# sean-lo/OptimalMatrixCompletion.jl

Hardware: AMD Instinct MI355X
Metric: B&B node-relaxations/sec, 100x100 k=1 (higher is better)
Workload: dtype f64

## Files before the change

### optimalmatrixcompletion.jl_amd/csrc/omc_device.h

```cpp
#ifndef OMC_DEVICE_H
#define OMC_DEVICE_H
#include <hip/hip_runtime.h>
#include <stdint.h>

#define ROW_TRACE 0
#define ROW_BOX 1
#define ROW_BOUND 2
#define ROW_CUT 3

#define CONE_CLIP01 0
#define CONE_EVALS 2
#define CONE_SEP 3
#define CONE_TOPK 4
#define CONE_BIG 5
#define SMALL_PROJ 0
#define SMALL_RECOVER 1

#define OMC_ST_OPTIMAL 0
#define OMC_ST_SLOW 1
#define OMC_ST_TIME 2
#define OMC_ST_INFEASIBLE 3

#include "omc_layout.h"

struct OmcWS {
  int nB;
  int B, Btot, n, m, k, nnz, Rmax, Lmax, breakpoints, rmax, stall_checks, np16, max_sweeps, max_iters;
  int *node_of, *init, *fin;
  const int* slot_list;
  int check_every, early_stop_after; double early_stop_factor;
  double *gap_prev, *gap_rate; int* slow_votes;
  const double* rho_node;
  double *oY, *oU, *oalphaX, *obx, *oobj, *olb, *olmin, *orho; int *ostatus, *oiters;
  double gamma, rho, rho_f_ratio, relax, eps_gap, eps_feas, sumA2;
  double* rho_b;
  double* bfac;
  int *nbump, *lastbump;
  int bump_max, bump_after, bump_gap; double bump_ratio, bump_factor;
  const int* col_ptr;
  const int* col_idx;
  const double* col_val;
  const double* Ncnt;
  const int* row_ptr;
  const int* row_idx;
  double* lamD;
  double* lamDX;
  const double* wY1;
  double *Y, *Yp;
  double* U;
  double *D1, *D3;
  double *W1, *E3;
  int* w1_fac;
  int skip_yp;
  double* Qb;
  int* rr;
  double *Vt, *D3V, *W3V, *Q3V;
  double *D3T, *W3T, *Q3T;
  double* dS;
  double *alpha, *alphaX;
  double* sval;
  double *objcol, *c0col;
  double* Mchk;
  int check_xs;
  double *Mbuf, *Vrow;
  double* fro2;
  int* vvalid;
  double *MbufC, *VrowC, *fro2c; int* vvalidC; int ws_mode;
  int sub_enable, sub_qmax, sub_chunk, sub_debug; double sub_tol, sub_adapt;
  double* sub_zscratch;
  double* Xs;
  double* sub_theta;
  double* trM;
  double* V3; int* v3valid;
  int *sub_wait, *sub_nfail;
  int *sub_on, *cone_done;
  int* ws_first; int ws_phase;
  int* ws_need;
  int sub_guard;
  int* sep_done;
  int cert_enable; double *XsC, *sub_thetaC, *trMc, *lb_est; int *sub_onC, *confirm;
  int shor;
  int shN;
  const double *shP0, *shD0;
  double clip_hi;
  double inv_s2;
  const int *load_from, *save_to;
  double *pY, *pD1, *pD3, *pU, *palpha, *psval, *pXs, *ptheta, *pscal;
  int mw_budget; int* mw_stat; double* ev_out;
  int* pmw_stat;
  int* sub_stat;
  int* R;
  int *rkind, *rcut, *rbi, *rbj;
  double* rcoef;
  double* rrhs;
  double* cutx;
  double* G;
  int setup_gram_inline;
  double* lam;
  double *obj, *objout, *objprev, *lbprev, *lb, *c0, *evsum, *cpen, *cst, *rp, *rd, *lmin;
  double* bx;
  int *done, *status, *iters, *sweeps, *stall;
  int* rowov;
  OmcGeom geo;
  double* cp_scratch;
  int cp_pair; int cp_nsolo; const int* cp_solo;
  int cp_nwide; const int* cp_wide;
  int cp_nrest;
  int cp_nblock, cp_nslab; const int *cp_block, *cp_slab; const unsigned char* cp_isblock; double* cp_bslab; int* cp_nfact;
  double* Yx;
  int cone_512;
  int cp_series;
  int cp_maxpass;
  int cp_xcd;
  double *cone_scratch, *glob_scratch, *small_scratch;
  double* chk_scratch;
  double* stamps;
  int accel, aa_mem, aa_every, aa_start, aa_dim;
  double aa_reg, aa_safeguard;
  double *aa_F, *aa_G, *aa_zin;
  double* aa_fn;
  int *aa_hist, *aa_head, *aa_pending, *aa_valid, *aa_nacc, *aa_nrej;
  int *cert_flag, *cert_have;
  double *cb_rho, *cbLam, *cblam, *cbPsi, *cbBound;
  double *ocLam, *oclam, *ocPsi, *ocBound; int* ocHave;
};
// ... 45 lines not shown
```

### optimalmatrixcompletion.jl_amd/csrc/omc_device.hip

```cpp
#include <hip/hip_runtime.h>
#include <type_traits>
#include <stdint.h>
#include "omc_device.h"
#include "omc.h"

#include "omc_wave.h"


#ifdef OMC_STAMPS
#define STAMP(slot) do { __syncthreads(); if (blockIdx.x == 0 && threadIdx.x == 0) { long long t_ = __builtin_amdgcn_s_memtime(); w.stamps[slot] += (double)(t_ - t_prev_); t_prev_ = t_; } } while (0)
#define STAMP_BEGIN() long long t_prev_ = __builtin_amdgcn_s_memtime()
#define DIAG_T0() long long t_diag0_ = __builtin_amdgcn_s_memtime()
#define DIAG_ADD(cls, b, v) atomicAdd(&w.stamps[32 + (size_t)(cls) * w.B + (b)], (double)(v))
#define DIAG_CYC(cls, b) DIAG_ADD(cls, b, __builtin_amdgcn_s_memtime() - t_diag0_)
#define WSTAMP_BEGIN() long long tw_prev_ = __builtin_amdgcn_s_memtime()
#define WSTAMP_BEGIN2() tw_prev_ = __builtin_amdgcn_s_memtime()
#define WSTAMP(slot) do { if (b == 0 && j == 0 && lane == 0) { long long t_ = __builtin_amdgcn_s_memtime(); w.stamps[slot] += (double)(t_ - tw_prev_); tw_prev_ = t_; } } while (0)
#else
#define WSTAMP_BEGIN() do {} while (0)
#define WSTAMP_BEGIN2() do {} while (0)
#define WSTAMP(slot) do {} while (0)
#define STAMP(slot) do {} while (0)
#define STAMP_BEGIN() do {} while (0)
#define DIAG_T0() do {} while (0)
// ... 1485 lines not shown
    while ((r + 1) * (r + 2) / 2 <= tile) ++r;
    ti[t] = r; tj[t] = tile - r * (r + 1) / 2;
    const int ia = (ti[t] << 4) + li, jb = (tj[t] << 4) + li;
    ma[t] = (ia < n) ? 1.0 : 0.0; mb[t] = (jb < n) ? 1.0 : 0.0;
    La[t] = L + ((ia < n) ? ia : n - 1);
    Lb[t] = L + ((jb < n) ? jb : n - 1);
    acc[t] = double4v{0.0, 0.0, 0.0, 0.0};
  }
  if (m4 >= 16) {
#pragma unroll
    for (int t = 0; t < NT; ++t)
#pragma unroll
      for (int u = 0; u < 4; ++u) { aq[t][u] = La[t][(size_t)(4 * u + lk) * n]; bq[t][u] = Lb[t][(size_t)(4 * u + lk) * n]; }
  }
  int k0 = 0;
  for (; k0 + 16 <= m4; k0 += 16) {
#pragma unroll
    for (int u = 0; u < 4; ++u) {
      int kn = k0 + 16 + 4 * u + lk;
      kn = (kn < m4) ? kn : kn - 16;
#pragma unroll
      for (int t = 0; t < NT; ++t) {
        const double a = aq[t][u] * ma[t], bv = bq[t][u] * mb[t];
        aq[t][u] = La[t][(size_t)kn * n]; bq[t][u] = Lb[t][(size_t)kn * n];
        acc[t] = __builtin_amdgcn_mfma_f64_16x16x4f64(a, bv, acc[t], 0, 0, 0);
      }
    }
  }
  for (; k0 < m; k0 += 4) {
    const int kk = k0 + lk;
#pragma unroll
    for (int t = 0; t < NT; ++t) {
      const double a = (kk < m) ? La[t][(size_t)kk * n] * ma[t] : 0.0, bv = (kk < m) ? Lb[t][(size_t)kk * n] * mb[t] : 0.0;
      acc[t] = __builtin_amdgcn_mfma_f64_16x16x4f64(a, bv, acc[t], 0, 0, 0);
    }
  }
#pragma unroll
  for (int t = 0; t < NT; ++t)
#pragma unroll
    for (int r = 0; r < 4; ++r) {
      const int i = (ti[t] << 4) + lk + 4 * r, j = (tj[t] << 4) + li;
      if (i < n && j < n && i >= j) store(i, j, acc[t][r]);
    }
}
template <int NT, class StoreF>
__device__ __forceinline__ void mfma_LLt(const double* L, int n, int m, StoreF store) {
  const int tid = threadIdx.x, wv = tid >> 6, lane = tid & 63, nw = blockDim.x >> 6, li = lane & 15, lk = lane >> 4;
  const int nt = (n + 15) >> 4, ntile = nt * (nt + 1) / 2;
  int tile = wv;
  for (; tile + (NT - 1) * nw < ntile; tile += NT * nw) mfma_LLt_tiles<NT>(L, n, m, tile, nw, li, lk, store);
  if constexpr (NT > 1) for (; tile < ntile; tile += nw) mfma_LLt_tiles<1>(L, n, m, tile, nw, li, lk, store);
}

template <bool USE_LDS>
__global__ void __launch_bounds__(256) k_small(OmcWS w, int mode) {
  extern __shared__ double smem[];
  __shared__ double red[32];
  __shared__ int s_cnt, s_nsel;
  __shared__ double s_base;
  const int b = slot_of(w, blockIdx.x), tid = threadIdx.x, T = blockDim.x;
  if (w.done[b] && mode == SMALL_PROJ) return;
  if (mode == SMALL_RECOVER && !w.fin[b]) return;
  const int nb = w.node_of[b];
  const int n = w.n, k = w.k, rm = w.rmax;
  const int r = w.rr[nb];
  const int N3 = (mode == SMALL_PROJ) ? r + k : r;
  const int Np = (N3 + 1) & ~1, ld = Np | 1;
  auto base = [&]() { if constexpr (USE_LDS) return (double*)smem; else return w.small_scratch + (size_t)b * w.geo.small.slab_stride; }();
  const SmallLayout L = small_layout(n, rm, k);
  const int ld3 = L.ld3;
  double* T1 = base;
  double* M3 = base + L.M3;
  double *Gm = base + L.Gm, *ev = base + L.ev, *wgt = base + L.wgt;
  int* sel = (int*)(base + L.sel);
  double* Cc = base + L.Cc;
  double* Qs = base + L.Qs;
  const double* Q = w.Qb + (size_t)nb * n * rm;
  const double* Y = w.Y + (size_t)b * n * n;
  const double* D3 = w.D3 + (size_t)b * n * n;
  const double* Vt = w.Vt + (size_t)b * rm * k;
  STAMP_BEGIN();
  DIAG_T0();
  constexpr int T1_RS = 16;
  if (USE_LDS && r <= T1_RS && n <= T) {
    for (int e = tid; e < n * T1_RS; e += T) { const int j = e / T1_RS, a = e % T1_RS; Qs[e] = (a < r) ? Q[(size_t)a * n + j] : 0.0; }
    __syncthreads();
    {
      const int wv_ = tid >> 6, lane_ = tid & 63, li = lane_ & 15, lk = lane_ >> 4, nt = (n + 15) >> 4, nw_ = T >> 6;
      const bool proj = (mode == SMALL_PROJ);
      for (int ti = wv_; ti < nt; ti += nw_) {
        const int ia = (ti << 4) + li; const bool va = ia < n; const int iac = va ? ia : 0;
        double4v acc = {0.0, 0.0, 0.0, 0.0};
        double ya[4], da[4];
#pragma unroll
        for (int u = 0; u < 4; ++u) { const int kk = 4 * u + lk, kc = (kk < n) ? kk : 0; ya[u] = Y[(size_t)kc * n + iac]; da[u] = proj ? D3[(size_t)kc * n + iac] : 0.0; }
        for (int k0 = 0; k0 < n; k0 += 16) {
#pragma unroll
          for (int u = 0; u < 4; ++u) {
            const int kk = k0 + 4 * u + lk; const bool vk = kk < n;
            const double av = ya[u] - da[u], bv = Qs[(vk ? kk : 0) * T1_RS + li];
            const int kn = kk + 16, knc = (kn < n) ? kn : 0;
            ya[u] = Y[(size_t)knc * n + iac]; da[u] = proj ? D3[(size_t)knc * n + iac] : 0.0;
            acc = __builtin_amdgcn_mfma_f64_16x16x4f64((va && vk) ? av : 0.0, vk ? bv : 0.0, acc, 0, 0, 0);
          }
        }
#pragma unroll
        for (int r4 = 0; r4 < 4; ++r4) {
          const int row = (ti << 4) + lk + 4 * r4;
          if (row < n && li < r) T1[(size_t)li * n + row] = acc[r4];
        }
      }
      __syncthreads();
    }
  } else {
    for (int e = tid; e < n * r; e += T) {
      int i = e % n, a = e / n;
      double acc = 0.0;
      if (mode == SMALL_PROJ) for (int j = 0; j < n; ++j) acc += (Y[(size_t)j * n + i] - D3[(size_t)j * n + i]) * Q[(size_t)a * n + j];
      else for (int j = 0; j < n; ++j) acc += Y[(size_t)j * n + i] * Q[(size_t)a * n + j];
      T1[(size_t)a * n + i] = acc;
    }
    __syncthreads();
  }
  STAMP(16);
  for (int e = tid; e < N3 * N3; e += T) {
    int i = e % N3, j = e / N3;
    double v;
    if (i < r && j < r) { v = 0.0; for (int t = 0; t < n; ++t) v += Q[(size_t)i * n + t] * T1[(size_t)j * n + t]; }
    else if (i < r) v = Vt[(size_t)(j - r) * rm + i] - w.D3V[(size_t)b * rm * k + (size_t)(j - r) * rm + i];
    else if (j < r) v = Vt[(size_t)(i - r) * rm + j] - w.D3V[(size_t)b * rm * k + (size_t)(i - r) * rm + j];
    else v = ((i == j) ? 1.0 : 0.0) - w.D3T[(size_t)b * k * k + (size_t)(j - r) * k + (i - r)];
    M3[(size_t)j * ld3 + i] = v;
  }
  __syncthreads();
  STAMP(17);
  if (N3 == 0) return;
// ... 47 lines not shown
        for (int c2 = 0; c2 < r; ++c2) dot += gt[c2] * Vt[(size_t)j * rm + c2];
        acc += wgt[s] * gt[a] * dot;
      }
      Cc[(size_t)j * rm + a] = acc;
    }
    __syncthreads();
    for (int e = tid; e < n * k; e += T) {
      int i = e % n, j = e / n;
      double acc = 0.0;
      for (int a = 0; a < r; ++a) acc += T1[(size_t)a * n + i] * Cc[(size_t)j * rm + a];
      w.U[(size_t)b * n * k + e] = acc;
    }
    return;
  }
  STAMP(18);
  if (tid == 0) {
    int npos = 0, nneg = 0;
    for (int t = 0; t < N3; ++t) { double lamv = sqrt(ev[t]) - sigma; if (lamv > 0.0) ++npos; else if (lamv < 0.0) ++nneg; }
    const bool use_neg = nneg <= npos;
    int c = 0;
    for (int t = 0; t < N3; ++t) {
      double nu2 = ev[t], lamv = sqrt(nu2) - sigma;
      if (use_neg ? (lamv < 0.0) : (lamv > 0.0)) { sel[c] = t; wgt[c] = fabs(lamv) / nu2; ++c; }
    }
    s_nsel = c; s_base = use_neg ? 1.0 : 0.0;
  }
  __syncthreads();
  const bool acc_is_Q3 = (s_base == 1.0);
  double* dS = w.dS + (size_t)b * rm * rm;
  auto store = [&](int i, int j, double v, double Mv) {
    double accv = v - s_base * Mv;
    double q3 = acc_is_Q3 ? accv : (accv - Mv);
    double p3 = acc_is_Q3 ? (Mv + accv) : accv;
    if (i < r && j < r) { dS[(size_t)j * rm + i] = q3; dS[(size_t)i * rm + j] = q3; }
    else if (i >= r && j < r) {
      w.W3V[(size_t)b * rm * k + (size_t)(i - r) * rm + j] = p3;
      w.Q3V[(size_t)b * rm * k + (size_t)(i - r) * rm + j] = q3;
    } else if (i >= r && j >= r) {
      w.W3T[(size_t)b * k * k + (size_t)(j - r) * k + (i - r)] = p3; w.W3T[(size_t)b * k * k + (size_t)(i - r) * k + (j - r)] = p3;
      w.Q3T[(size_t)b * k * k + (size_t)(j - r) * k + (i - r)] = q3; w.Q3T[(size_t)b * k * k + (size_t)(i - r) * k + (j - r)] = q3;
    }
  };
  spectral_rebuild(Gm, ld, N3, sel, wgt, s_nsel, s_base, entry, store);
  __syncthreads();
  __threadfence_block();
  STAMP(19);
  for (int e = tid; e < n * r; e += T) {
    int i = e % n, a = e / n;
    double acc = 0.0;
    for (int c2 = 0; c2 < r; ++c2) acc += Q[(size_t)c2 * n + i] * dS[(size_t)a * rm + c2];
    T1[(size_t)a * n + i] = acc;
  }
  __syncthreads();
  double* E3 = w.E3 + (size_t)b * n * n;
  if (USE_LDS && r <= 16 && n <= T) {
    const int wv_ = tid >> 6, lane_ = tid & 63, li = lane_ & 15, lk = lane_ >> 4, nt = (n + 15) >> 4, nw_ = T >> 6;
    for (int tile = wv_; tile < nt * nt; tile += nw_) {
      const int ti = tile / nt, tj = tile - ti * nt;
      const int ia = (ti << 4) + li, jb = (tj << 4) + li;
      const bool va = ia < n, vb = jb < n;
      const int iac = va ? ia : 0, jbc = vb ? jb : 0;
      double4v acc = {0.0, 0.0, 0.0, 0.0};
#pragma unroll
      for (int k0 = 0; k0 < 16; k0 += 4) {
        const int a = k0 + lk; const bool vk = a < r;
        const double av = T1[(size_t)(vk ? a : 0) * n + iac], bv = Qs[jbc * 16 + a];
        acc = __builtin_amdgcn_mfma_f64_16x16x4f64((va && vk) ? av : 0.0, vb ? bv : 0.0, acc, 0, 0, 0);
      }
#pragma unroll
      for (int r4 = 0; r4 < 4; ++r4) {
        const int row = (ti << 4) + lk + 4 * r4, col = (tj << 4) + li;
        if (row < n && col < n) E3[(size_t)row * n + col] = acc[r4];
      }
    }
  } else {
    for (int e = tid; e < n * n; e += T) {
      int i = e % n, j = e / n;
      if (i < j) continue;
      double acc = 0.0;
      for (int a = 0; a < r; ++a) acc += T1[(size_t)a * n + i] * Q[(size_t)a * n + j];
      E3[(size_t)j * n + i] = acc; E3[(size_t)i * n + j] = acc;
    }
  }
  STAMP(20);
  if (tid == 0) DIAG_CYC(5, b);
}

__device__ __forceinline__ double w1_entry(const double* Xf, const double* wf, int nf, int n, int i, int j) {
  const int p = (i > j) ? i : j, q = (i > j) ? j : i;
  double acc = 0.0;
  for (int c = 0; c < nf; ++c) { const double* x = Xf + (size_t)c * n; acc += x[p] * (x[q] * wf[c]); }
  return acc;
}

template <bool USE_LDS>
__global__ void __launch_bounds__(512) k_global(OmcWS w) {
  extern __shared__ double smem[];
  __shared__ double red[32];
  __shared__ double s_Gp[NNQP_GP_DOUBLES];
  __shared__ double s_sv[NNQP_PMAX], s_tmp[NNQP_PMAX];
  __shared__ int s_pl[NNQP_PMAX];
  const int b = slot_of(w, blockIdx.x), tid = threadIdx.x, T = blockDim.x;
  if (w.done[b]) return;
  const int nb = w.node_of[b];
  const int n = w.n, k = w.k, m = w.m, rm = w.rmax;
  const GlobLayout L = glob_layout(n, k, rm, w.Rmax);
// ... 1115 lines not shown
```

### optimalmatrixcompletion.jl_amd/csrc/omc_host.h

```cpp
#pragma once
#include <hip/hip_runtime.h>
#include <stdint.h>
#include <atomic>
#include <mutex>
#include <string>
#include <thread>
#include <unordered_map>
#include <vector>

#include "omc.h"
#include "omc_carve.h"
#include "omc_device.h"
#include "omc_shor_relax.h"
#include "omc_shor_index.h"
#include "omc_walks.h"

extern thread_local std::string g_err;
static inline int fail(int code, const std::string& msg) { g_err = msg; return code; }
#define HIPCHK(x)                                                                                         \
  do {                                                                                                    \
    hipError_t e_ = (x);                                                                                  \
    if (e_ != hipSuccess) {                                                                               \
      g_err = std::string(#x) + ": " + hipGetErrorString(e_);                                             \
      return (int)e_ > 0 ? (int)e_ : 999;                                                                 \
// ... 40 lines not shown
  field = (T*)b.p;
  return 0;
}
template <class T> static inline int bind(DevBuf& b, T*& field, size_t count, hipStream_t zero_on) {
  const int rc = bind(b, field, count);
  if (rc) return rc;
  HIPCHK(hipMemsetAsync(b.p, 0, count * sizeof(T), zero_on));
  return 0;
}
#define BIND(...) do { int r_ = bind(__VA_ARGS__); if (r_) return r_; } while (0)

struct PinBuf {
  void* p = nullptr; size_t cap = 0;
  PinBuf() = default;
  PinBuf(const PinBuf&) = delete;
  PinBuf& operator=(const PinBuf&) = delete;
  ~PinBuf() { if (p) (void)hipHostFree(p); }
  int ensure(size_t bytes) {
    if (bytes <= cap) return 0;
    if (p) (void)hipHostFree(p);
    p = nullptr; cap = 0;
    hipError_t e = hipHostMalloc(&p, bytes, hipHostMallocDefault);
    if (e != hipSuccess) { g_err = std::string("hipHostMalloc: ") + hipGetErrorString(e); return (int)e; }
    cap = bytes;
    return 0;
  }
  template <class T> T* as() { return (T*)p; }
};

struct Tuning {
  bool altmin_nolds = false;
  bool colprox_no_xcd = false;
  bool cone_512 = false;
  bool dense_proj = false;
  bool host_phases = false;
  bool global_nolds = false;
  bool no_colprox_pair = false;
  bool no_graph = false;
  bool no_subspace = false;
  bool no_ws_split = false;
  bool segv_trace = false;
  bool setup_gram_inline = false;
  bool shor_explicit = false;
  bool shor_no_subspace = false;
  int check_xs = 16;
  int colprox_block_min = 65;
  int cone_multi_min = 1025;
  int event_merge = 1;
  int graph_max = 16;
  int harvest_async = 1;
  int harvest_async_min_live = 256;
  int plain_multi_min = 1025;
  int shor_index_device_min = 0;
  int shor_select_kb = 1048576;
  int streams = 4;
  int sub_debug = 0;
  int sub_qmax = 24;
  int timing_stride = 1;
  int ws_quiet = 1;
};
struct Knob { const char* name; bool Tuning::*flag; int Tuning::*num; };
inline const Knob OMC_KNOBS[] = {
  {"OMC_ALTMIN_NOLDS", &Tuning::altmin_nolds, nullptr},      {"OMC_COLPROX_NO_XCD", &Tuning::colprox_no_xcd, nullptr},
  {"OMC_CONE_512", &Tuning::cone_512, nullptr},              {"OMC_DENSE_PROJ", &Tuning::dense_proj, nullptr},
  {"OMC_GLOBAL_NOLDS", &Tuning::global_nolds, nullptr},      {"OMC_HOST_PHASES", &Tuning::host_phases, nullptr},
  {"OMC_NO_COLPROX_PAIR", &Tuning::no_colprox_pair, nullptr},
  {"OMC_NO_GRAPH", &Tuning::no_graph, nullptr},              {"OMC_NO_SUBSPACE", &Tuning::no_subspace, nullptr},
  {"OMC_NO_WS_SPLIT", &Tuning::no_ws_split, nullptr},        {"OMC_SEGV_TRACE", &Tuning::segv_trace, nullptr},
  {"OMC_SETUP_GRAM_INLINE", &Tuning::setup_gram_inline, nullptr},
  {"OMC_SHOR_EXPLICIT", &Tuning::shor_explicit, nullptr},    {"OMC_SHOR_NO_SUBSPACE", &Tuning::shor_no_subspace, nullptr},
  {"OMC_COLPROX_BLOCK_MIN", nullptr, &Tuning::colprox_block_min},
  {"OMC_CHECK_XS", nullptr, &Tuning::check_xs},              {"OMC_CONE_MULTI_MIN", nullptr, &Tuning::cone_multi_min},
  {"OMC_EVENT_MERGE", nullptr, &Tuning::event_merge},
  {"OMC_GRAPH_MAX", nullptr, &Tuning::graph_max},            {"OMC_SHOR_SELECT_KB", nullptr, &Tuning::shor_select_kb},
  {"OMC_SHOR_INDEX_DEVICE_MIN", nullptr, &Tuning::shor_index_device_min},
  {"OMC_HARVEST_ASYNC", nullptr, &Tuning::harvest_async},    {"OMC_HARVEST_ASYNC_MIN_LIVE", nullptr, &Tuning::harvest_async_min_live},
  {"OMC_WS_QUIET", nullptr, &Tuning::ws_quiet},
  {"OMC_STREAMS", nullptr, &Tuning::streams},                {"OMC_PLAIN_MULTI_MIN", nullptr, &Tuning::plain_multi_min},
  {"OMC_SUB_DEBUG", nullptr, &Tuning::sub_debug},            {"OMC_SUB_QMAX", nullptr, &Tuning::sub_qmax},
  {"OMC_TIMING_STRIDE", nullptr, &Tuning::timing_stride},
};

struct omc_instance {
  int n = 0, m = 0, k = 0, device = 0, nnz = 0, cmax = 0;
  double gamma = 0, sumA2 = 0;
  std::vector<int> col_ptr, col_idx; std::vector<double> col_val;
  std::vector<double> A; std::vector<uint8_t> mask;
  std::vector<double> Ncnt;
  std::vector<int> row_ptr, row_idx; std::vector<double> row_val;
  DevBuf drow_ptr, drow_idx, drow_val, aR, arkind, arcut, arbi, arbj, arcoef, arrhs, acutx, aU0, aU, aV, aobj, aint, aG, aG2;
  hipStream_t stream = nullptr;
  Tuning tun;
  hipStream_t gs[3] = {};
  hipEvent_t gev[5] = {};
  hipEvent_t gevc[5] = {};
  hipEvent_t ev_main = nullptr;
  PinBuf pin_flags[2], pin_list[2], pin_done, pin_jobs; DevBuf bgramjobs;
  hipEvent_t ev_up[4] = {}; bool ev_up_rec[4] = {}; hipEvent_t ev_gram = nullptr; bool ev_gram_rec = false;
  double host_ms[OMC_HOST_NPHASE] = {0}; int64_t host_cnt[OMC_HOST_NPHASE] = {0};
  DevBuf dA, dmask, dcol_ptr, dcol_idx, dcol_val, dNcnt, dwY, dsolo, dwide;
  int nwide = 0;
  int nsolo = 0;
  DevBuf dblock, dslab, disblock, bcpb, bnfact;
  int nblock = 0, nslab = 0, nrest = 0, cpb_cl = 0, cpb_cs = 0, crest_max = 0;
  bool lists_valid = false; int lists_block_min = 0; bool lists_pair = true;
  DevBuf bYx, bY, bYp, bU, bD1, bD3, bW1, bE3, bQb, brr, bsm, bdS, balpha, balphaX, bsval, bMchk, bsmall, bchk;
  DevBuf bR, brkind, brcut, brbi, brbj, brcoef, brrhs, bcutx, bG, blam;
  DevBuf bobjcol, baaF, baaG, baaZ, baaS, baaI, bMbufC, bVrowC, bchkS, bchkI;
  DevBuf bslotlist, bgap, bvotes, blamDX, bXsC, bsubSC, bsubIC;
  DevBuf bsubz, bscal, bbx, bint, bcp, bcone, bglob, bXout, bThout, bXin, bMbuf, bVrow, bXs, bsubS, bsubI;
  long long sub_tot[8] = {0};
  DevBuf bmwstat, sbigmw, pjM, pjV, pjW, pjS, pjD, pjI;
  long long mw_tot[5] = {0};
  DevBuf bpmwstat; long long pmw_tot[4] = {0};
  OmcWS ws{};
  omc_relax_params params{};
  bool staged = false;
  double last_solve_seconds = 0; long long total_sweeps = 0; int last_iters_total = 0;
  std::thread worker; std::atomic<int> worker_running{0}, nodes_done{0}; int worker_rc = 0; std::string worker_err;
  int reserve_nodes = 0, reserve_cuts = 0, node_cap = 0, staged_cut_type = 0; std::atomic<int> Btot_live{0}; bool append_closed = true; std::mutex append_mu; hipStream_t append_stream = nullptr;
  std::atomic<int> hold{0};
  std::vector<int> done_q; size_t done_read = 0; std::mutex done_mu; hipStream_t fetch_stream = nullptr;
  void* comm = nullptr; int comm_rank = 0, comm_world = 1; DevBuf bcomm, amobj; int amobj_B = 0;
  int wall_khz = 0;
  std::vector<double> rho_scale_per_node; DevBuf brho, brhon, blamD, bslotint, boY, boU, boal, bobx, boscal, boint;
  int Btot = 0;
  bool keep_cert = false; DevBuf bcbD, bcbI, bocD, bocI;
  bool keep_shor_cert = false; DevBuf scbD, socD, socNq;
  DevBuf dbD, dbI, dbM, dbS, dbL;
  DevBuf sdD, sdI, sdGi, sdGb, sdGr; double sdb_ms = 0.0;
  DevBuf sbits, scb, scx, scz, soff, stot, sout, shi, slo, sexist, shist, sohi, solo, scnt;
  bool shor_ready = false; int shor_W = 0; long long shor_pairs = 0;
// ... 26 lines not shown
```

### optimalmatrixcompletion.jl_amd/csrc/omc_layout.h

```cpp
#ifndef OMC_LAYOUT_H
#define OMC_LAYOUT_H
#include <hip/hip_runtime.h>
#include <stddef.h>

#define NNQP_PMAX 64
#define NNQP_GP_DOUBLES (NNQP_PMAX * (NNQP_PMAX + 1) / 2)
#define NNQP_STATIC_BYTES ((NNQP_GP_DOUBLES + 2 * NNQP_PMAX) * 8 + NNQP_PMAX * 4)
#define OMC_MAX_DYN_LDS (144 * 1024)
#define SUBP 16
#define GL_XS 16
#define OMC_HD __host__ __device__ inline
struct ConeLayout { int Np, ld; size_t ev, wgt, sel; };
OMC_HD ConeLayout cone_carve(int N, int ld) { const int Np = (N + 1) & ~1; const size_t ev = (size_t)Np * ld; return {Np, ld, ev, ev + Np, ev + 2 * Np}; }
OMC_HD ConeLayout cone_layout(int N) { return cone_carve(N, ((N + 1) & ~1) | 1); }
OMC_HD size_t cone_bytes(int N) { const ConeLayout L = cone_layout(N); return L.sel * 8 + (size_t)L.Np * 4 + 16; }
OMC_HD size_t ws_bytes(int N, int ld) { const ConeLayout L = cone_carve(N, ld); return (L.sel + L.Np) * 8 + (size_t)(L.Np + 2) * 4 + 64; }
OMC_HD int ws_rpl(int N, int lpp) { return (((N + lpp - 1) / lpp) + 1) & ~1; }
struct WsGeometry { int lpp, rpl, ld, use_lds; size_t bytes; };
OMC_HD WsGeometry ws_geometry(int N) {
  const int Np2 = (N + 1) & ~1;
  int lpp = 16; while (lpp > 4 && lpp * (Np2 / 2) > 512) lpp >>= 1;
  int rpl = ws_rpl(N, lpp), Nrp = rpl * lpp;
  int ld = Nrp + ((16 - (Nrp & 31)) & 31);
  if (ws_bytes(N, ld) > OMC_MAX_DYN_LDS) ld = Nrp + 2;
  const int use_lds = ws_bytes(N, ld) <= OMC_MAX_DYN_LDS;
  if (!use_lds) {
    lpp = 16; rpl = ws_rpl(N, 16);
    if (rpl > 32 && N <= 1024) { lpp = 64; rpl = ws_rpl(N, 64); }
    ld = rpl * lpp + 2;
  }
  return {rpl <= 32 ? lpp : 0, rpl, ld, use_lds, ws_bytes(N, ld)};
}
#define GRAM_CHUNK 8
#define CB_XS 4096
OMC_HD int gram_npairs(int R) { return R * (R + 1) / 2; }
OMC_HD int gram_chunks(int R) { return (gram_npairs(R) + GRAM_CHUNK - 1) / GRAM_CHUNK; }
OMC_HD void gram_pair_of(int p, int R, int* r, int* s) {
  int rr = 0;
  while (p >= R - rr) { p -= R - rr; ++rr; }
  *r = rr; *s = rr + p;
}
OMC_HD void gram_pair_next(int R, int* r, int* s) { if (++*s == R) { ++*r; *s = *r; } }
#define MW_B 16
#define MW_MAXSW 32
#define MW_MIN_ORDER 145
#define MW_MAX_ORDER 4096
#define MW_TAU_PLAIN 1e-14
#define MW_PLAIN_SWEEPS 30
struct MwLayout { int ld, Ncp, nb; size_t ev, lam, wgt, sel, smax, head, bytes, fro; };
OMC_HD MwLayout mw_layout(int N) {
  const int NP = (N + 15) & ~15, Ncp = (N + 2 * MW_B - 1) & ~(2 * MW_B - 1), ld = NP + 4;
  static_assert(2 * MW_B >= 16, "fro: the NP / 16 partial sums of the plain sequence lie in the Ncp words of wgt, NP <= Ncp");
  const size_t ev = (size_t)Ncp * ld, sel = ev + 3 * (size_t)Ncp, smax = sel + Ncp / 2, head = smax + MW_MAXSW;
  return {ld, Ncp, Ncp / MW_B, ev, ev + Ncp, ev + 2 * (size_t)Ncp, sel, smax, head, (head + 4) * 8, ev + 2 * (size_t)Ncp};
}
OMC_HD int mw_plain_launches(const MwLayout& L, int sweeps) { return sweeps * (L.nb - 1) + 4; }
struct SubLayout { int LD, zglob; size_t Za, Cs, Hs, Gj, th, evj, red, wgt, sel, bytes; };
OMC_HD SubLayout sub_layout(int np16) {
  const int LD = np16 + 2, zglob = np16 > 512; const size_t blk = (size_t)SUBP * LD, Cs = (zglob ? 1 : 2) * blk, th = Cs + 4 * 256 + 2 * 16 * 17;
  return {LD, zglob, blk, Cs, Cs + 4 * 256, Cs + 4 * 256 + 16 * 17, th, th + 16, th + 32, th + 64, th + 80, (th + 80 + 8) * 8};
}
#define SMALL_STATIC_LDS 1024
struct SmallLayout { int ld3; size_t M3, Gm, ev, wgt, sel, Cc, Qs, bytes; };
OMC_HD SmallLayout small_layout(int n, int rmax, int k) {
  const int ld3 = rmax + k, Npm = (ld3 + 1) & ~1, ldm = Npm | 1;
  const size_t M3 = (size_t)n * rmax, Gm = M3 + (size_t)ld3 * ld3, ev = Gm + (size_t)Npm * ldm, sel = ev + 2 * Npm, Cc = sel + Npm / 2, Qs = Cc + (size_t)rmax * k + 2;
  return {ld3, M3, Gm, ev, ev + Npm, sel, Cc, Qs, (Qs + (size_t)n * 16) * 8 + 104};
}
#define GLOB_STATIC_LDS ((size_t)NNQP_STATIC_BYTES + 2560)
struct GlobLayout { size_t tU, tV, cvec, mu, xs, qrow, bytes; };
OMC_HD GlobLayout glob_layout(int n, int k, int rmax, int Rmax) {
  const size_t tU = (size_t)n * (n + 1) / 2, tV = tU + (size_t)n * k, cvec = tV + (size_t)rmax * k, xs = cvec + 2 * Rmax, qrow = xs + (size_t)GL_XS * n;
  return {tU, tV, cvec, cvec + Rmax, xs, qrow, (qrow + Rmax) * 8 + 80};
}
OMC_HD bool glob_w1_fits(int n) { return (size_t)SUBP * n <= (size_t)NNQP_GP_DOUBLES; }
struct CpRegLayout { int Lm, vo, pinv, sidx, doubles; };
OMC_HD CpRegLayout cp_reg_layout(int c, int keepB) { const int tri = (c * (c + 1)) >> 1, vo = (keepB ? 2 : 1) * tri; return {keepB ? tri : 0, vo, vo + c, vo + 2 * c, vo + 4 * c + 8}; }
struct CpBodyLayout { size_t Lm, va, vy, vz, vo, doubles; };
OMC_HD CpBodyLayout cp_body_layout(int c) { const size_t tri = (size_t)c * (c + 1) / 2, va = 2 * tri; return {tri, va, va + c, va + 2 * c, va + 3 * c, va + 4 * c + 8}; }
#define CPB_TILE 256
#define CPB_STATIC_LDS 4352
struct CpBlockLayout { int nb, ntiles; size_t panel, va, vy, vz, vw, vo, sidx, doubles, slab; };
OMC_HD int cpb_tile(int I, int J) { return ((I * (I + 1)) >> 1) + J; }
OMC_HD CpBlockLayout cp_block_layout(int c, int lds) {
  const int nb = c > 0 ? (c + 15) >> 4 : 1, nt = (nb * (nb + 1)) >> 1;
  const size_t cp = (size_t)16 * nb, va = (size_t)CPB_TILE * (lds ? nt : (nb > 1 ? nb - 1 : 1));
  return {nb, nt, 0, va, va + cp, va + 2 * cp, va + 3 * cp, va + 4 * cp, va + 5 * cp, va + 5 * cp + cp / 2, lds ? 0 : (size_t)CPB_TILE * nt};
}
OMC_HD int cp_block_fits(int c, int lds) { return cp_block_layout(c, lds).doubles * 8 <= (size_t)OMC_MAX_DYN_LDS; }
OMC_HD int cp_block_lds_cmax() { int nb = 1; while (cp_block_fits(16 * (nb + 1), 1)) ++nb; return 16 * nb; }
OMC_HD int cp_block_cmax() { int nb = 1; while (cp_block_fits(16 * (nb + 1), 0)) ++nb; return 16 * nb; }
OMC_HD void cp_block_plan(int cmax, int block_min, long long* out) {
  const int ldsc = cp_block_lds_cmax(), on = cmax >= block_min && cmax >= 1 && cmax <= cp_block_cmax();
  const CpBlockLayout L = cp_block_layout(cmax, cmax <= ldsc);
  out[0] = ldsc; out[1] = on ? (long long)(L.doubles * 8) : 0; out[2] = on ? (long long)L.slab : 0;
  out[3] = on ? (long long)((160 * 1024) / (L.doubles * 8 + CPB_STATIC_LDS)) : 0; out[4] = on;
}
struct Altmin1Layout { size_t v, h, g, u0, cvec, mu, bytes; };
OMC_HD Altmin1Layout altmin1_layout(int n, int m, int Rmax) { const size_t h = (size_t)n + m, cvec = h + 3 * n; return {(size_t)n, h, h + n, h + 2 * n, cvec, cvec + Rmax, (cvec + 2 * Rmax + 8) * 8}; }
struct AltminKLayout { size_t ut, u0, g, H, Hinv, v, cvec, mu, bytes; };
OMC_HD AltminKLayout altmink_layout(int n, int m, int k, int Rmax) {
  const size_t nk = (size_t)n * k, H = 4 * nk, v = H + 2 * nk * k, cvec = v + (size_t)k * m;
  return {nk, 2 * nk, 3 * nk, H, H + nk * k, v, cvec, cvec + Rmax, (cvec + 2 * Rmax + 8) * 8};
}
struct AltminWLayout { size_t ut, u0, g, H, Hinv, v, cvec, mu, th, th2, q, qt, step, tmp, act, J, P, Lc, bytes; };
OMC_HD AltminWLayout altminw_layout(int n, int m, int k, int Rmax) {
  const size_t nk = (size_t)n * k, mq = (size_t)k * k, H = 4 * nk, v = H + 2 * nk * k, cvec = v + (size_t)k * m, th = cvec + 2 * Rmax, J = th + 7 * mq, Lc = J + 2 * mq * mq;
  return {nk, 2 * nk, 3 * nk, H, H + nk * k, v, cvec, cvec + Rmax, th, th + mq, th + 2 * mq, th + 3 * mq, th + 4 * mq, th + 5 * mq, th + 6 * mq, J, J + mq * mq, Lc,
          (Lc + mq * (mq + 1) / 2 + 8) * 8};
}
struct KernelPlan { int use_lds; size_t lds_bytes, slab_stride; };
OMC_HD KernelPlan plan_block(size_t bytes, bool fits) { return {fits ? 1 : 0, fits ? bytes : 0, fits ? 0 : bytes / 8 + 8}; }
#define ALTMIN_KMAX 8
OMC_HD int altmin_variant(int k) { return k == 1 ? 1 : (k <= 4 ? 2 : 3); }
OMC_HD KernelPlan altmin_plan(int n, int m, int k, int Rmax, int nolds) {
  const int var = altmin_variant(k);
  const size_t bytes = (var == 1) ? altmin1_layout(n, m, Rmax).bytes : (var == 2) ? altmink_layout(n, m, k, Rmax).bytes : altminw_layout(n, m, k, Rmax).bytes;
  return plan_block(bytes, bytes + 8 * 1024 <= ((var == 1) ? (size_t)OMC_MAX_DYN_LDS - 8 * 1024 : (size_t)128 * 1024) && !nolds);
}
struct OmcGeom {
// ... 46 lines not shown
```

### optimalmatrixcompletion.jl_amd/csrc/omc_relax_solve.cpp

```cpp
#include <algorithm>
#include <chrono>
#include <stdio.h>

#include "omc_events.h"
#include "omc_host.h"
#include "omc_slots.h"

static_assert(SLOT_HARVEST_NONE == OMC_HARVEST_NONE && SLOT_HARVEST_SYNC == OMC_HARVEST_SYNC && SLOT_HARVEST_ASYNC == OMC_HARVEST_ASYNC, "omc_slots.h restates the plans of omc.h");

namespace {

using Clock = std::chrono::steady_clock;

int sum_sub_stat(int* sub_stat, int S, long long tot[8], hipStream_t s) {
  std::vector<int> ss(8 * (size_t)S);
  HIPCHK(hipMemcpyAsync(ss.data(), sub_stat, sizeof(int) * ss.size(), hipMemcpyDeviceToHost, s));
  HIPCHK(hipStreamSynchronize(s));
  for (int q = 0; q < 8; ++q) tot[q] = 0;
  for (int b = 0; b < S; ++b) for (int q = 0; q < 8; ++q) tot[q] += ss[8 * b + q];
  HIPCHK(hipMemsetAsync(sub_stat, 0, sizeof(int) * ss.size(), s));
  return 0;
}

enum { T_S = 0, T_M = 1, T_B = 2, T_C = 3, T_NSTREAM = 4 };
// ... 119 lines not shown
    tape.touch(T_S);
    if (nlist) { HIPCHK(hipMemcpyAsync(h->bslotlist.p, alist, sizeof(int) * nlist, hipMemcpyHostToDevice, s)); HIPCHK(hipEventRecord(h->ev_up[2 + q], s)); h->ev_up_rec[2 + q] = true; }
    return 0;
  }

  int gram_launch(int njobs) {
    if (tun.setup_gram_inline || njobs <= 0) return 0;
    for (int q = 0; q < njobs; ++q)
      if (jobs[2 * q] < 0 || jobs[2 * q] >= S || jobs[2 * q + 1] < 0 || jobs[2 * q + 1] >= Btot) return fail(OMC_ERR_ARGUMENT, "omc_relax_solve: k_setup_gram job outside the slots / nodes");
    HIPCHK(hipMemcpyAsync(h->bgramjobs.p, jobs, sizeof(int) * 2 * (size_t)njobs, hipMemcpyHostToDevice, sb));
    tape.touch(ib);
    TIMED_ON(ib, OMC_KERNEL_SETUP, false, 0, omc_launch_setup_gram(&w, h->bgramjobs.as<int>(), njobs, Btot, sb));
    HIPCHK(hipEventRecord(h->ev_gram, sb)); h->ev_gram_rec = true;
    tape.touch(ib);
    return 0;
  }
  int gram_jobs_free() {
    if (h->ev_gram_rec) { HIPCHK(hipEventSynchronize(h->ev_gram)); h->ev_gram_rec = false; }
    return 0;
  }
  int gram_join() {
    if (h->ev_gram_rec && sb != s) { HIPCHK(hipStreamWaitEvent(s, h->ev_gram, 0)); tape.touch(T_S); }
    return 0;
  }
  int setup_slots(int units) {
    tape.touch(T_S);
    if (shor && std::find(starts.begin(), starts.end(), it) == starts.end()) starts.push_back(it);
    if (shor) omc_shor_launch_setup(&sw, s);
    TIMED(OMC_KERNEL_SETUP, units, omc_launch_setup(&w, s));
    { int rc = gram_join(); if (rc) return rc; }
    mw_budget[0] = mw_budget[1] = MAX_SWEEPS;
    quiet = quiet_next = false;
    return 0;
  }

  int prepare() {
    for (int c = 0; c < OMC_KERNEL_NCLASS; ++c) { h->launches[c] = 0; h->ms[c] = 0; h->units[c] = 0; }
    tape.reset();
    for (int q = 0; q < OMC_HOST_NPHASE; ++q) { h->host_ms[q] = 0; h->host_cnt[q] = 0; }
    for (int q = 0; q < 2; ++q) { int rc = h->pin_flags[q].ensure(sizeof(int) * 3 * (size_t)S); if (rc) return rc; rc = h->pin_list[q].ensure(sizeof(int) * (size_t)S); if (rc) return rc; }
    { int rc = h->pin_done.ensure(sizeof(int) * ((size_t)S + 1)); if (rc) return rc; rc = h->pin_jobs.ensure(sizeof(int) * 2 * (size_t)S); if (rc) return rc; rc = h->bgramjobs.ensure(sizeof(int) * 2 * (size_t)S); if (rc) return rc; }
    for (int q = 0; q < 4; ++q) { if (!h->ev_up[q]) HIPCHK(hipEventCreateWithFlags(&h->ev_up[q], hipEventDisableTiming)); h->ev_up_rec[q] = false; }
    if (!h->ev_gram) HIPCHK(hipEventCreateWithFlags(&h->ev_gram, hipEventDisableTiming));
    h->ev_gram_rec = false;
    if (multi && !h->ev_main) {
      for (hipStream_t& q : h->gs) HIPCHK(hipStreamCreateWithFlags(&q, hipStreamNonBlocking));
      for (int q = 0; q < 5; ++q) { HIPCHK(hipEventCreateWithFlags(&h->gev[q], hipEventDisableTiming)); HIPCHK(hipEventCreateWithFlags(&h->gevc[q], hipEventDisableTiming)); }
      HIPCHK(hipEventCreateWithFlags(&h->ev_main, hipEventDisableTiming));
    }
    sm = multi ? h->gs[0] : s; sb = multi ? h->gs[1] : s; sc = multi ? h->gs[2] : s;
    if (multi) { im = T_M; ib = T_B; ic = T_C; }
    hip_events.st[T_S] = s; hip_events.st[T_M] = sm; hip_events.st[T_B] = sb; hip_events.st[T_C] = sc;
    h->ws.setup_gram_inline = tun.setup_gram_inline ? 1 : 0;
    h->ws.check_xs = std::min(std::max(0, tun.check_xs), CB_XS);
    done = h->pin_done.as<int>(); jobs = h->pin_jobs.as<int>();
    book = SlotBook(S, jobs, done);
    int rc = gram_launch(book.start(Btot)); if (rc) return rc;
    rc = push_flags(false); if (rc) return rc;
    if (book.active() < S) { HIPCHK(hipMemcpyAsync(w.done, done, sizeof(int) * S, hipMemcpyHostToDevice, s)); HIPCHK(hipStreamSynchronize(s)); }
    rc = setup_slots(S); if (rc) return rc;
    rc = push_list(); if (rc) return rc;
    h->total_sweeps = 0;
    graph_max = Btot <= tun.graph_max ? tun.graph_max : 0;
    mw_any = w.geo.mw || w.geo.plain_mw || (shor && h->wbig.geo.mw);
    for (int q = 0; q < 5; ++q) h->mw_tot[q] = 0;
    for (int q = 0; q < 4; ++q) h->pmw_tot[q] = 0;
    split_solve = multi && !tun.no_ws_split && w.sub_enable && w.geo.ws_lpp && w.ws_first;
    return 0;
  }

  int refill_idle() {
    if (book.next_node() >= Btot) return 0;
    int rc = gram_jobs_free(); if (rc) return rc;
    const int ninit = book.refill_idle(Btot);
    if (!ninit) return 0;
    rc = gram_launch(ninit); if (rc) return rc;
    rc = push_flags(false); if (rc) return rc;
    rc = setup_slots(ninit); if (rc) return rc;
    rc = push_list(); if (rc) return rc;
    wait_main = true;
    return 0;
  }

  int close_unslotted(int st) {
    const int first = book.close_unslotted(Btot);
    if (first >= Btot) return 0;
    const size_t c = (size_t)(Btot - first);
    std::vector<int> stv(c, st), itz(c, 0);
    std::vector<double> inf(c, 1e300), ninf(c, -1e300);
    HIPCHK(hipMemcpyAsync(w.ostatus + first, stv.data(), sizeof(int) * c, hipMemcpyHostToDevice, s));
    HIPCHK(hipMemcpyAsync(w.oiters + first, itz.data(), sizeof(int) * c, hipMemcpyHostToDevice, s));
    HIPCHK(hipMemcpyAsync(w.oobj + first, inf.data(), 8 * c, hipMemcpyHostToDevice, s));
    HIPCHK(hipMemcpyAsync(w.olb + first, ninf.data(), 8 * c, hipMemcpyHostToDevice, s));
    HIPCHK(hipStreamSynchronize(s));
    return 0;
  }

  int run_dry(bool* ended) {
    *ended = false;
    {
      std::lock_guard<std::mutex> lk(h->append_mu);
      Btot = h->Btot_live.load();
      if (timed_out) { int rc = close_unslotted(OMC_ST_TIME); if (rc) return rc; }
      if (book.next_node() >= Btot && (!h->hold.load() || elapsed() > P.time_limit)) { h->append_closed = true; *ended = true; return 0; }
    }
    if (book.next_node() >= Btot) { std::this_thread::sleep_for(std::chrono::microseconds(100)); return 0; }
// ... 337 lines not shown
```

Before: 2385.

## Add fused small-projection chain path with prefetched MFMA T1 and warm-started Jacobi

Adds a dedicated SMALL_PROJ path in k_small that runs the whole small PSD projection in one specialised routine. It prefetches Y and D3 tiles in registers for an MFMA-based T1 product, warm-starts the 16-wide Jacobi eigensolver from the previous node's eigenvectors, and does eigenvalue selection with wave ballots instead of a serial thread. The aim is to cut global-load latency, serial sections and eigensolver sweeps in the small projection kernel. It enlarges the LDS layout by a scratch region and adds per-slot V3 state, which can go stale between nodes and affect convergence.

```diff
diff --git a/optimalmatrixcompletion.jl_amd/csrc/omc_device.h b/optimalmatrixcompletion.jl_amd/csrc/omc_device.h
--- a/optimalmatrixcompletion.jl_amd/csrc/omc_device.h
+++ b/optimalmatrixcompletion.jl_amd/csrc/omc_device.h
@@ -71,6 +71,7 @@
   double* Xs;
   double* sub_theta;
   double* trM;
+  int small_chain;
   double* V3; int* v3valid;
   int *sub_wait, *sub_nfail;
   int *sub_on, *cone_done;
diff --git a/optimalmatrixcompletion.jl_amd/csrc/omc_device.hip b/optimalmatrixcompletion.jl_amd/csrc/omc_device.hip
--- a/optimalmatrixcompletion.jl_amd/csrc/omc_device.hip
+++ b/optimalmatrixcompletion.jl_amd/csrc/omc_device.hip
@@ -1561,6 +1561,231 @@
   if constexpr (NT > 1) for (; tile < ntile; tile += nw) mfma_LLt_tiles<1>(L, n, m, tile, nw, li, lk, store);
 }
 
+#define SMALL_T1_NC 1
+template <bool TWO>
+__device__ __forceinline__ void small_T1_tiles(const double* Y, const double* D3, const double* Qs, double* T1, int n, int r, int t0, int t1, int li, int lk,
+                                               double (&ya)[2][4 * SMALL_T1_NC], double (&da)[2][4 * SMALL_T1_NC]) {
+  constexpr int NT = TWO ? 2 : 1;
+  const int tt[2] = {t0, t1};
+  bool va[2]; int iac[2];
+#pragma unroll
+  for (int t = 0; t < NT; ++t) { const int ia = (tt[t] << 4) + li; va[t] = ia < n; iac[t] = va[t] ? ia : 0; }
+  double4v acc[2] = {{0.0, 0.0, 0.0, 0.0}, {0.0, 0.0, 0.0, 0.0}};
+  for (int k0 = 0; k0 < n; k0 += 16 * SMALL_T1_NC) {
+#pragma unroll
+    for (int c = 0; c < SMALL_T1_NC; ++c) {
+      if (c > 0 && k0 + 16 * c >= n) break;
+#pragma unroll
+      for (int u = 0; u < 4; ++u) {
+        const int kk = k0 + 16 * c + 4 * u + lk; const bool vk = kk < n;
+        const double bv = Qs[(vk ? kk : 0) * 16 + li];
+        const int kn = kk + 16 * SMALL_T1_NC, knc = (kn < n) ? kn : 0;
+#pragma unroll
+        for (int t = 0; t < NT; ++t) {
+          const double av = ya[t][4 * c + u] - da[t][4 * c + u];
+          ya[t][4 * c + u] = Y[(size_t)knc * n + iac[t]]; da[t][4 * c + u] = D3[(size_t)knc * n + iac[t]];
+          acc[t] = __builtin_amdgcn_mfma_f64_16x16x4f64((va[t] && vk) ? av : 0.0, vk ? bv : 0.0, acc[t], 0, 0, 0);
+        }
+      }
+    }
+  }
+#pragma unroll
+  for (int t = 0; t < NT; ++t)
+#pragma unroll
+    for (int r4 = 0; r4 < 4; ++r4) {
+      const int row = (tt[t] << 4) + lk + 4 * r4;
+      if (row < n && li < r) T1[(size_t)li * n + row] = acc[t][r4];
+    }
+}
+__device__ __forceinline__ void small_select_wave(double ev_t, double sigma, int N3, int* sel, double* wgt, int* s_nsel, double* s_base) {
+  const int t = threadIdx.x & 63;
+  const bool valid = t < N3;
+  const double lamv = sqrt(ev_t) - sigma;
+  const unsigned long long pos = __ballot(valid && lamv > 0.0), neg = __ballot(valid && lamv < 0.0);
+  const bool use_neg = __popcll(neg) <= __popcll(pos);
+  const unsigned long long m = use_neg ? neg : pos;
+  if ((m >> t) & 1ull) { const int c = __popcll(m & ((1ull << t) - 1ull)); sel[c] = t; wgt[c] = fabs(lamv) / ev_t; }
+  if (t == 0) { *s_nsel = __popcll(m); *s_base = use_neg ? 1.0 : 0.0; }
+}
+__device__ __forceinline__ void small_proj_chain(const OmcWS& w, int b, int nb, double* base, double* red, int* s_cnt, int* s_nsel, double* s_base) {
+  const int tid = threadIdx.x, T = blockDim.x, wv = tid >> 6, lane = tid & 63, li = lane & 15, lk = lane >> 4, nw = T >> 6;
+  const int n = w.n, k = w.k, rm = w.rmax;
+  const int r = w.rr[nb];
+  const int N3 = r + k;
+  const int Np = (N3 + 1) & ~1, ld = Np | 1, nt = (n + 15) >> 4;
+  const SmallLayout L = small_layout(n, rm, k);
+  const int ld3 = L.ld3;
+  double* T1 = base;
+  double* M3 = base + L.M3;
+  double *Gm = base + L.Gm, *ev = base + L.ev, *wgt = base + L.wgt;
+  int* sel = (int*)(base + L.sel);
+  double* Qs = base + L.Qs;
+  double *Ss = base + L.Cs, *Vs = base + L.Cs + 256, *dSs = base + L.Cs;
+  const double* Q = w.Qb + (size_t)nb * n * rm;
+  const double* Y = w.Y + (size_t)b * n * n;
+  const double* D3 = w.D3 + (size_t)b * n * n;
+  const double* Vt = w.Vt + (size_t)b * rm * k;
+  const bool wave16 = Np <= 16;
+  double* Vp = w.V3 + (size_t)b * 256;
+  const bool warm = wave16 && w.v3valid[b] != 0;
+  STAMP_BEGIN();
+  DIAG_T0();
+  double ya[2][4 * SMALL_T1_NC], da[2][4 * SMALL_T1_NC];
+  auto first_chunk = [&](int t, int tile) {
+    const int ia = (tile << 4) + li, iac = (ia < n) ? ia : 0;
+#pragma unroll
+    for (int u = 0; u < 4 * SMALL_T1_NC; ++u) { const int kk = 4 * u + lk, kc = (kk < n) ? kk : 0; ya[t][u] = Y[(size_t)kc * n + iac]; da[t][u] = D3[(size_t)kc * n + iac]; }
+  };
+  if (wv < nt) first_chunk(0, wv);
+  if (wv + nw < nt) first_chunk(1, wv + nw);
+  const double vprev = (warm && tid < 256) ? Vp[tid] : 0.0;
+  {
+    const int qd = T / n, qr = T - qd * n;
+    int a = tid / n, j = tid - a * n;
+    for (int e = tid; e < n * 16; e += T) {
+      Qs[j * 16 + a] = (a < r) ? Q[(size_t)a * n + j] : 0.0;
+      a += qd; j += qr; if (j >= n) { j -= n; ++a; }
+    }
+  }
+  __syncthreads();
+  for (int tb = wv; tb < nt; tb += 2 * nw) {
+    const bool two = tb + nw < nt;
+    if (tb != wv) { first_chunk(0, tb); if (two) first_chunk(1, tb + nw); }
+    if (two) small_T1_tiles<true>(Y, D3, Qs, T1, n, r, tb, tb + nw, li, lk, ya, da);
+    else small_T1_tiles<false>(Y, D3, Qs, T1, n, r, tb, tb, li, lk, ya, da);
+  }
+  __syncthreads();
+  STAMP(16);
+  for (int e = tid; e < N3 * N3; e += T) {
+    int i = e % N3, j = e / N3;
+    double v;
+    if (i < r && j < r) { v = 0.0; for (int t = 0; t < n; ++t) v += Qs[t * 16 + i] * T1[(size_t)j * n + t]; }
+    else if (i < r) v = Vt[(size_t)(j - r) * rm + i] - w.D3V[(size_t)b * rm * k + (size_t)(j - r) * rm + i];
+    else if (j < r) v = Vt[(size_t)(i - r) * rm + j] - w.D3V[(size_t)b * rm * k + (size_t)(i - r) * rm + j];
+    else v = ((i == j) ? 1.0 : 0.0) - w.D3T[(size_t)b * k * k + (size_t)(j - r) * k + (i - r)];
+    M3[(size_t)j * ld3 + i] = v;
+  }
+  __syncthreads();
+  STAMP(17);
+  auto entry = [&](int i, int j) { return M3[(size_t)j * ld3 + i]; };
+  double sigma;
+  if (wave16) {
+    if (tid < 256) Vs[tid] = vprev;
+    double fro = 0.0;
+    for (int e = tid; e < N3 * N3; e += T) { const int i = e % N3, j = e / N3; const double v = 0.5 * (entry(i, j) + entry(j, i)); fro += v * v; Ss[j * 16 + i] = v; }
+    fro = sqrt(block_sum(fro, red));
+    sigma = 1.5 * fro + 1e-300;
+    for (int e = tid; e < Np * Np; e += T) {
+      const int i = e % Np, t = e / Np;
+      double v = 0.0;
+      if (i < N3 && t < N3) {
+        if (warm) { for (int j = 0; j < N3; ++j) v += (Ss[j * 16 + i] + ((i == j) ? sigma : 0.0)) * Vs[t * 16 + j]; }
+        else v = Ss[t * 16 + i] + ((i == t) ? sigma : 0.0);
+      }
+      Gm[(size_t)t * ld + i] = v;
+    }
+    __syncthreads();
+    STAMP(30);
+    if (tid < WAVE) {
+      jacobi_sweeps_wave16(Gm, ev, N3, Np, ld, 1e-14, 30);
+      WAVE_SYNC();
+      double a = 0.0;
+      if (tid < N3) { for (int i = 0; i < N3; ++i) { const double x = Gm[(size_t)tid * ld + i]; a += x * x; } ev[tid] = a; }
+      small_select_wave(a, sigma, N3, sel, wgt, s_nsel, s_base);
+    }
+    __syncthreads();
+    for (int e = tid; e < N3 * N3; e += T) { const int i = e % N3, t = e / N3; Vp[t * 16 + i] = Gm[(size_t)t * ld + i] * rsqrt(ev[t]); }
+    if (tid == 0) w.v3valid[b] = 1;
+  } else {
+    sigma = eig_frontend(Gm, ev, N3, Np, ld, entry, red, s_cnt, nullptr);
+    if (N3 <= WAVE) { if (tid < WAVE) small_select_wave((tid < N3) ? ev[tid] : 0.0, sigma, N3, sel, wgt, s_nsel, s_base); }
+    else if (tid == 0) {
+      int npos = 0, nneg = 0;
+      for (int t = 0; t < N3; ++t) { double lamv = sqrt(ev[t]) - sigma; if (lamv > 0.0) ++npos; else if (lamv < 0.0) ++nneg; }
+      const bool use_neg = nneg <= npos;
+      int c = 0;
+      for (int t = 0; t < N3; ++t) {
+        double nu2 = ev[t], lamv = sqrt(nu2) - sigma;
+        if (use_neg ? (lamv < 0.0) : (lamv > 0.0)) { sel[c] = t; wgt[c] = fabs(lamv) / nu2; ++c; }
+      }
+      *s_nsel = c; *s_base = use_neg ? 1.0 : 0.0;
+    }
+    __syncthreads();
+  }
+  STAMP(18);
+  const double sb = *s_base;
+  const bool acc_is_Q3 = (sb == 1.0);
+  double* dS = w.dS + (size_t)b * rm * rm;
+  auto store = [&](int i, int j, double v, double Mv) {
+    double accv = v - sb * Mv;
+    double q3 = acc_is_Q3 ? accv : (accv - Mv);
+    double p3 = acc_is_Q3 ? (Mv + accv) : accv;
+    if (i < r && j < r) { dS[(size_t)j * rm + i] = q3; dS[(size_t)i * rm + j] = q3; dSs[j * 16 + i] = q3; dSs[i * 16 + j] = q3; }
+    else if (i >= r && j < r) {
+      w.W3V[(size_t)b * rm * k + (size_t)(i - r) * rm + j] = p3;
+      w.Q3V[(size_t)b * rm * k + (size_t)(i - r) * rm + j] = q3;
+    } else if (i >= r && j >= r) {
+      w.W3T[(size_t)b * k * k + (size_t)(j - r) * k + (i - r)] = p3; w.W3T[(size_t)b * k * k + (size_t)(i - r) * k + (j - r)] = p3;
+      w.Q3T[(size_t)b * k * k + (size_t)(j - r) * k + (i - r)] = q3; w.Q3T[(size_t)b * k * k + (size_t)(i - r) * k + (j - r)] = q3;
+    }
+  };
+  {
+    const int nsel = *s_nsel;
+    for (int e = tid; e < N3 * N3; e += T) {
+      const int i = e % N3, j = e / N3;
+      if (i < j) continue;
+      double acc = 0.0;
+      for (int s = 0; s < nsel; ++s) { const double* gt = Gm + (size_t)sel[s] * ld; const double gj = gt[j] * wgt[s]; acc += gt[i] * gj; }
+      const double Mv = entry(i, j);
+      store(i, j, sb * Mv + acc, Mv);
+    }
+  }
+  __syncthreads();
+  STAMP(19);
+  {
+    const int a = tid & 15;
+    double dcol[16];
+#pragma unroll
+    for (int c2 = 0; c2 < 16; ++c2) dcol[c2] = (c2 < r && a < r) ? dSs[c2 * 16 + a] : 0.0;
+    if (a < r)
+      for (int i = tid >> 4; i < n; i += T >> 4) {
+        double q[16];
+#pragma unroll
+        for (int c2 = 0; c2 < 16; ++c2) q[c2] = Qs[i * 16 + c2];
+        double acc = 0.0;
+#pragma unroll
+        for (int c2 = 0; c2 < 16; ++c2) if (c2 < r) acc += q[c2] * dcol[c2];
+        T1[(size_t)a * n + i] = acc;
+      }
+  }
+  __syncthreads();
+  STAMP(29);
+  double* E3 = w.E3 + (size_t)b * n * n;
+  for (int tj = wv; tj < nt; tj += nw) {
+    const int jb = (tj << 4) + li; const bool vb = jb < n; const int jbc = vb ? jb : 0;
+    double bq[4];
+#pragma unroll
+    for (int u = 0; u < 4; ++u) { const double bv = Qs[jbc * 16 + 4 * u + lk]; bq[u] = vb ? bv : 0.0; }
+    for (int ti = 0; ti < nt; ++ti) {
+      const int ia = (ti << 4) + li; const bool va = ia < n; const int iac = va ? ia : 0;
+      double4v acc = {0.0, 0.0, 0.0, 0.0};
+#pragma unroll
+      for (int u = 0; u < 4; ++u) {
+        const int a = 4 * u + lk; const bool vk = a < r;
+        const double av = T1[(size_t)(vk ? a : 0) * n + iac];
+        acc = __builtin_amdgcn_mfma_f64_16x16x4f64((va && vk) ? av : 0.0, bq[u], acc, 0, 0, 0);
+      }
+#pragma unroll
+      for (int r4 = 0; r4 < 4; ++r4) {
+        const int row = (ti << 4) + lk + 4 * r4, col = (tj << 4) + li;
+        if (row < n && col < n) E3[(size_t)row * n + col] = acc[r4];
+      }
+    }
+  }
+  STAMP(20);
+  if (tid == 0) DIAG_CYC(5, b);
+}
+
 template <bool USE_LDS>
 __global__ void __launch_bounds__(256) k_small(OmcWS w, int mode) {
   extern __shared__ double smem[];
@@ -1588,9 +1813,12 @@
   const double* Y = w.Y + (size_t)b * n * n;
   const double* D3 = w.D3 + (size_t)b * n * n;
   const double* Vt = w.Vt + (size_t)b * rm * k;
+  constexpr int T1_RS = 16;
+  if constexpr (USE_LDS) {
+    if (w.small_chain && mode == SMALL_PROJ && r <= T1_RS && n <= T && N3 > 0) { small_proj_chain(w, b, nb, base, red, &s_cnt, &s_nsel, &s_base); return; }
+  }
   STAMP_BEGIN();
   DIAG_T0();
-  constexpr int T1_RS = 16;
   if (USE_LDS && r <= T1_RS && n <= T) {
     for (int e = tid; e < n * T1_RS; e += T) { const int j = e / T1_RS, a = e % T1_RS; Qs[e] = (a < r) ? Q[(size_t)a * n + j] : 0.0; }
     __syncthreads();
@@ -1744,6 +1972,7 @@
     T1[(size_t)a * n + i] = acc;
   }
   __syncthreads();
+  STAMP(29);
   double* E3 = w.E3 + (size_t)b * n * n;
   if (USE_LDS && r <= 16 && n <= T) {
     const int wv_ = tid >> 6, lane_ = tid & 63, li = lane_ & 15, lk = lane_ >> 4, nt = (n + 15) >> 4, nw_ = T >> 6;
diff --git a/optimalmatrixcompletion.jl_amd/csrc/omc_host.h b/optimalmatrixcompletion.jl_amd/csrc/omc_host.h
--- a/optimalmatrixcompletion.jl_amd/csrc/omc_host.h
+++ b/optimalmatrixcompletion.jl_amd/csrc/omc_host.h
@@ -116,6 +116,7 @@
   int harvest_async_min_live = 256;
   int plain_multi_min = 1025;
   int shor_index_device_min = 0;
+  int small_chain = 1;
   int shor_select_kb = 1048576;
   int streams = 4;
   int sub_debug = 0;
@@ -142,6 +143,7 @@
   {"OMC_WS_QUIET", nullptr, &Tuning::ws_quiet},
   {"OMC_STREAMS", nullptr, &Tuning::streams},                {"OMC_PLAIN_MULTI_MIN", nullptr, &Tuning::plain_multi_min},
   {"OMC_SUB_DEBUG", nullptr, &Tuning::sub_debug},            {"OMC_SUB_QMAX", nullptr, &Tuning::sub_qmax},
+  {"OMC_SMALL_CHAIN", nullptr, &Tuning::small_chain},
   {"OMC_TIMING_STRIDE", nullptr, &Tuning::timing_stride},
 };
 
diff --git a/optimalmatrixcompletion.jl_amd/csrc/omc_layout.h b/optimalmatrixcompletion.jl_amd/csrc/omc_layout.h
--- a/optimalmatrixcompletion.jl_amd/csrc/omc_layout.h
+++ b/optimalmatrixcompletion.jl_amd/csrc/omc_layout.h
@@ -61,11 +61,13 @@
   return {LD, zglob, blk, Cs, Cs + 4 * 256, Cs + 4 * 256 + 16 * 17, th, th + 16, th + 32, th + 64, th + 80, (th + 80 + 8) * 8};
 }
 #define SMALL_STATIC_LDS 1024
-struct SmallLayout { int ld3; size_t M3, Gm, ev, wgt, sel, Cc, Qs, bytes; };
+#define SMALL_CS 512
+struct SmallLayout { int ld3; size_t M3, Gm, ev, wgt, sel, Cc, Qs, Cs, bytes; };
 OMC_HD SmallLayout small_layout(int n, int rmax, int k) {
   const int ld3 = rmax + k, Npm = (ld3 + 1) & ~1, ldm = Npm | 1;
   const size_t M3 = (size_t)n * rmax, Gm = M3 + (size_t)ld3 * ld3, ev = Gm + (size_t)Npm * ldm, sel = ev + 2 * Npm, Cc = sel + Npm / 2, Qs = Cc + (size_t)rmax * k + 2;
-  return {ld3, M3, Gm, ev, ev + Npm, sel, Cc, Qs, (Qs + (size_t)n * 16) * 8 + 104};
+  const size_t Cs = Qs + (size_t)n * 16;
+  return {ld3, M3, Gm, ev, ev + Npm, sel, Cc, Qs, Cs, (Cs + SMALL_CS) * 8 + 104};
 }
 #define GLOB_STATIC_LDS ((size_t)NNQP_STATIC_BYTES + 2560)
 struct GlobLayout { size_t tU, tV, cvec, mu, xs, qrow, bytes; };
diff --git a/optimalmatrixcompletion.jl_amd/csrc/omc_relax_solve.cpp b/optimalmatrixcompletion.jl_amd/csrc/omc_relax_solve.cpp
--- a/optimalmatrixcompletion.jl_amd/csrc/omc_relax_solve.cpp
+++ b/optimalmatrixcompletion.jl_amd/csrc/omc_relax_solve.cpp
@@ -195,6 +195,7 @@
     if (multi) { im = T_M; ib = T_B; ic = T_C; }
     hip_events.st[T_S] = s; hip_events.st[T_M] = sm; hip_events.st[T_B] = sb; hip_events.st[T_C] = sc;
     h->ws.setup_gram_inline = tun.setup_gram_inline ? 1 : 0;
+    h->ws.small_chain = tun.small_chain ? 1 : 0;
     h->ws.check_xs = std::min(std::max(0, tun.check_xs), CB_XS);
     done = h->pin_done.as<int>(); jobs = h->pin_jobs.as<int>();
     book = SlotBook(S, jobs, done);
```

New measurement: 2441, median of 6. +2.4%, better.
